# 1005088h/3d_object_detection

Hardware: AMD Instinct MI355X
Metric: point-cloud frames/sec end-to-end (voxelise→NMS), eight_20cm, 1x MI355X (higher is better)
Workload: dtype f32; 1 GPU; configs/eight_20cm.json, synthetic KITTI-shape 64-beam 20k-point clouds (mean 20000 points, one distinct cloud per frame of a step), independent frames (batch=1 semantics), random-init weights (InstanceNorm backbone), AABB NMS; `value`: clouds resident in HBM; frames_per_pass_per_gpu=32, engine_max_batch=32, parallelism=frame-sharded x1

## Files before the change

### 3d_object_detection_amd/csrc/anchor_mask.hip

```cpp
#include "pp_common.h"

namespace {

__device__ __forceinline__ void occ_mark_body(const int32_t* __restrict__ coors, const int32_t* __restrict__ num_pillars,
                                                int gy, int32_t* __restrict__ occ)
{
    int p = blockIdx.x * blockDim.x + threadIdx.x;
    if (p >= *num_pillars) return;
    atomicAdd(&occ[coors[3 * p] * gy + coors[3 * p + 1]], 1);
}

__device__ __forceinline__ void scan_rows_body(int32_t* __restrict__ occ, int gx, int gy)
{
    int row = blockIdx.x * 4 + (threadIdx.x >> 6);
    int lane = threadIdx.x & 63;
    if (row >= gx) return;
    int32_t* r = occ + (size_t)row * gy;
    int carry = 0;
    constexpr int NB = 8;
    for (int yb = 0; yb < gy; yb += 64 * NB) {
        int vv[NB];
#pragma unroll
        for (int b = 0; b < NB; ++b) {
            const int y = yb + b * 64 + lane;
            const int x = r[y < gy ? y : gy - 1];
            vv[b] = y < gy ? x : 0;
        }
#pragma unroll
        for (int b = 0; b < NB; ++b) {
            const int y = yb + b * 64 + lane;
            int v = vv[b];
#pragma unroll
            for (int o = 1; o < 64; o <<= 1) {
                int t = __shfl_up(v, o);
                if (lane >= o) v += t;
            }
            v += carry;
            if (y < gy) r[y] = v;
            carry = __shfl(v, 63);
        }
    }
}

__device__ __forceinline__ void scan_cols_body(int32_t* __restrict__ occ, int gx, int gy)
{
    __shared__ int part[16][64];
    int lane = threadIdx.x & 63, w = threadIdx.x >> 6;
    int col = blockIdx.x * 64 + lane;
    int rows_per = (gx + 15) / 16;
    int x0 = w * rows_per, x1 = min(gx, x0 + rows_per);
    constexpr int CH = 16;
    int s = 0;
    if (col < gy)
        for (int x = x0; x < x1; x += CH) {
            int v[CH];
#pragma unroll
            for (int i = 0; i < CH; ++i) v[i] = occ[(size_t)min(x + i, x1 - 1) * gy + col];
#pragma unroll
            for (int i = 0; i < CH; ++i) s += (x + i < x1) ? v[i] : 0;
        }
    part[w][lane] = s;
    __syncthreads();
    int run = 0;
    for (int k = 0; k < w; ++k) run += part[k][lane];
    if (col < gy)
        for (int x = x0; x < x1; x += CH) {
            int v[CH];
#pragma unroll
            for (int i = 0; i < CH; ++i) v[i] = occ[(size_t)min(x + i, x1 - 1) * gy + col];
#pragma unroll
            for (int i = 0; i < CH; ++i)
                if (x + i < x1) {
                    run += v[i];
                    occ[(size_t)(x + i) * gy + col] = run;
                }
        }
}

__device__ __forceinline__ void mask_lookup_sep_body(const int32_t* __restrict__ sat, int gy, int H, int W, int types,
                                                       const int32_t* __restrict__ rect_x, const int32_t* __restrict__ rect_y,
                                                       uint8_t* __restrict__ mask)
{
    int64_t a = (int64_t)blockIdx.x * blockDim.x + threadIdx.x;
    int64_t total = (int64_t)types * H * W;
    if (a >= total) return;
    int iy = (int)(a % W);
    int64_t q = a / W;
    int ix = (int)(q % H);
    int t = (int)(q / H);
    int minx = rect_x[(t * H + ix) * 2], maxx = rect_x[(t * H + ix) * 2 + 1];
    int miny = rect_y[(t * W + iy) * 2], maxy = rect_y[(t * W + iy) * 2 + 1];
    int area = sat[maxx * gy + maxy] - sat[maxx * gy + miny] - sat[minx * gy + maxy] + sat[minx * gy + miny];
    mask[a] = area > 0;
}

__device__ __forceinline__ void mask_lookup_full_body(const int32_t* __restrict__ sat, int gy, int64_t A,
                                                        const int4* __restrict__ rects, uint8_t* __restrict__ mask)
{
    int64_t a = (int64_t)blockIdx.x * blockDim.x + threadIdx.x;
    if (a >= A) return;
    int4 r = rects[a];
    int area = sat[r.z * gy + r.w] - sat[r.z * gy + r.y] - sat[r.x * gy + r.w] + sat[r.x * gy + r.y];
    mask[a] = area > 0;
}

template <class Src> __global__ void __launch_bounds__(256) occ_mark(Src src, int gy)
{
    const pp_pre_frame F = src.get();
    occ_mark_body(F.coors, F.num, gy, F.occ);
}
template <class Src> __global__ void __launch_bounds__(256) scan_rows(Src src, int gx, int gy) { scan_rows_body(src.get().occ, gx, gy); }
template <class Src> __global__ void __launch_bounds__(1024) scan_cols(Src src, int gx, int gy) { scan_cols_body(src.get().occ, gx, gy); }
template <class Src> __global__ void __launch_bounds__(256) mask_lookup_sep(Src src, int gy, int H, int W, int types, const int32_t* __restrict__ rect_x,
                                                                            const int32_t* __restrict__ rect_y)
{
    const pp_pre_frame F = src.get();
    mask_lookup_sep_body(F.occ, gy, H, W, types, rect_x, rect_y, F.mask);
}
template <class Src> __global__ void __launch_bounds__(256) mask_lookup_full(Src src, int gy, int64_t A, const int4* __restrict__ rects)
{
    const pp_pre_frame F = src.get();
    mask_lookup_full_body(F.occ, gy, A, rects, F.mask);
}

}

template <class Src> static int anchor_mask_stages(pp_ctx* ctx, Src src, int g, hipStream_t stream)
{
    const int gx = ctx->gx, gy = ctx->gy;
    hipLaunchKernelGGL(occ_mark<Src>, dim3(pp_div_up(ctx->cfg.max_voxels, 256), 1, g), dim3(256), 0, stream, src, gy);
    hipLaunchKernelGGL(scan_rows<Src>, dim3(pp_div_up(gx, 4), 1, g), dim3(256), 0, stream, src, gx, gy);
    hipLaunchKernelGGL(scan_cols<Src>, dim3(pp_div_up(gy, 64), 1, g), dim3(1024), 0, stream, src, gx, gy);
    if (ctx->rect_separable) {
        int types = (int)(ctx->A / ((int64_t)ctx->H * ctx->W));
        hipLaunchKernelGGL(mask_lookup_sep<Src>, dim3(pp_div_up(ctx->A, 256), 1, g), dim3(256), 0, stream, src, gy, ctx->H, ctx->W, types,
                           ctx->rect_x, ctx->rect_y);
    } else {
        hipLaunchKernelGGL(mask_lookup_full<Src>, dim3(pp_div_up(ctx->A, 256), 1, g), dim3(256), 0, stream, src, gy, ctx->A, (const int4*)ctx->rects);
    }
    PP_HIP(hipGetLastError());
    return 0;
}

extern "C" int pp_anchor_mask(pp_ctx* ctx, const int32_t* coors, const int32_t* num_pillars, uint8_t* mask, void* stream_)
{
    if (!ctx) return PP_E_ARG;
    if (!coors || !num_pillars || !mask) return pp_fail(ctx, PP_E_ARG, "pp_anchor_mask: null pointer");
    if (ctx->A == 0) return pp_fail(ctx, PP_E_STATE, "pp_anchor_mask: call pp_set_anchors first");
    hipStream_t stream = (hipStream_t)stream_;
    pp_pre_frame f = {};
    PP_SET(f.coors, coors); PP_SET(f.num, num_pillars); PP_SET(f.mask, mask); PP_SET(f.occ, ctx->slot[0].occ);
    PP_HIP(hipMemsetAsync(ctx->slot[0].occ, 0, (size_t)ctx->gx * ctx->gy * sizeof(int32_t), stream));
    return anchor_mask_stages(ctx, pp_frames_one<pp_pre_frame>{f}, 1, stream);
}

int pp_anchor_mask_group(pp_ctx* ctx, int b0, int g, hipStream_t stream)
{
    return anchor_mask_stages(ctx, pp_frames_tab<pp_pre_frame>{ctx->d_pre + b0}, g, stream);
}
```

### 3d_object_detection_amd/csrc/pp_api.hip

```cpp
#include <cmath>
#include <cstdio>
#include <cstdlib>
#include <cstring>
#include "pp_common.h"

static std::string g_create_err;

int pp_fail_hip(pp_ctx* ctx, hipError_t e, const char* what, const char* file, int line)
{
    char buf[512];
    snprintf(buf, sizeof(buf), "%s failed: %s (%s:%d)", what, hipGetErrorString(e), file, line);
    if (ctx) ctx->err = buf; else g_create_err = buf;
    (void)hipGetLastError();
    return -(int)e;
}

int pp_fail(pp_ctx* ctx, int code, const char* msg)
{
    if (ctx) ctx->err = msg; else g_create_err = msg;
    return code;
}

extern "C" const char* pp_last_error(pp_ctx* ctx) { return ctx ? ctx->err.c_str() : g_create_err.c_str(); }
extern "C" int pp_version(void) { return 4; }

int pp_stage_mark(pp_ctx* ctx, hipStream_t stream, int id)
{
    if (!ctx->stage_on) return 0;
    if (ctx->stage_used >= ctx->stage_ev.size()) {
        hipEvent_t e;
        PP_HIP(hipEventCreate(&e));
        ctx->stage_ev.push_back(e);
        ctx->stage_id.push_back(-1);
        ctx->stage_stream.push_back(nullptr);
    }
    const hipError_t er = hipEventRecord(ctx->stage_ev[ctx->stage_used], stream);
    if (er != hipSuccess) { ctx->stage_on = false; ctx->stage_used = 0; return pp_fail_hip(ctx, er, "hipEventRecord(stage mark)", __FILE__, __LINE__); }
    ctx->stage_id[ctx->stage_used] = id;
    ctx->stage_stream[ctx->stage_used] = stream;
    ctx->stage_used++;
    return 0;
}

extern "C" int pp_stage_profile_begin(pp_ctx* ctx)
{
    if (!ctx) return PP_E_ARG;
    ctx->stage_on = true;
    ctx->stage_used = 0;
    return 0;
}

extern "C" int pp_stage_profile_end(pp_ctx* ctx, double* ms_h)
{
    if (!ctx || !ms_h) return PP_E_ARG;
    ctx->stage_on = false;
    const size_t used = ctx->stage_used;
    ctx->stage_used = 0;
    for (int i = 0; i < PP_ST_COUNT; ++i) ms_h[i] = 0.0;
    for (size_t i = 0; i + 1 < used; ++i) {
        const int id = ctx->stage_id[i];
        if (id < 0 || id >= PP_ST_COUNT) continue;
        if (ctx->stage_stream[i] != ctx->stage_stream[i + 1]) continue;
        PP_HIP(hipEventSynchronize(ctx->stage_ev[i]));
        PP_HIP(hipEventSynchronize(ctx->stage_ev[i + 1]));
        float ms = 0.f;
        PP_HIP(hipEventElapsedTime(&ms, ctx->stage_ev[i], ctx->stage_ev[i + 1]));
        ms_h[id] += ms;
    }
    return 0;
}

template <typename T>
static hipError_t dalloc(T** p, size_t count)
{
    return hipMalloc((void**)p, count * sizeof(T) + 256);
}

static int create_impl(pp_ctx* ctx)
{
    const pp_config& c = ctx->cfg;
    PP_HIP(hipSetDevice(ctx->device));
    size_t cells = (size_t)c.grid_size[0] * c.grid_size[1] * c.grid_size[2];
    size_t mp = (size_t)c.max_points;
    ctx->slot.resize(ctx->max_batch);
    for (int b = 0; b < ctx->max_batch; ++b) {
        pp_slot& S = ctx->slot[b];
        const size_t nslots = (size_t)c.max_voxels * c.max_num_points;
        PP_HIP(dalloc(&S.cell_first, cells + nslots + 4));
        S.slots = S.cell_first + cells;
        S.vox_scalars = S.slots + nslots;
        PP_HIP(dalloc(&S.pt_cell, mp));
        PP_HIP(dalloc(&S.pt_rank, mp));
        PP_HIP(dalloc(&S.wave_cnt, mp / 64 + 8));
        PP_HIP(dalloc(&S.occ, (size_t)ctx->gx * ctx->gy));
    }
    PP_HIP(hipMalloc((void**)&ctx->d_pre, sizeof(pp_pre_frame) * ctx->max_batch));
    PP_HIP(hipMalloc((void**)&ctx->d_post, sizeof(pp_post_frame) * ctx->max_batch));
    PP_HIP(dalloc(&ctx->pfn_w, 9 * 64));
    PP_HIP(dalloc(&ctx->pfn_scale, 64));
    PP_HIP(dalloc(&ctx->pfn_shift, 64));
    size_t mv = (size_t)c.max_voxels * ctx->max_batch;
    PP_HIP(dalloc(&ctx->f_voxels, mv * c.max_num_points * c.num_point_features));
    PP_HIP(dalloc(&ctx->f_coors, mv * 3));
    PP_HIP(dalloc(&ctx->f_npts, mv));
    PP_HIP(dalloc(&ctx->f_num, 4 * (size_t)ctx->max_batch));
    PP_HIP(dalloc(&ctx->f_feat, mv * 64));
    PP_HIP(dalloc(&ctx->f_canvas, (size_t)64 * ctx->gx * ctx->gy));
    PP_HIP(dalloc(&ctx->f_pmap, (size_t)ctx->max_batch * ctx->gx * ctx->gy));
    size_t HW = (size_t)ctx->H * ctx->W;
    size_t Amax = HW * c.num_anchor_per_loc * ctx->max_batch;
    PP_HIP(dalloc(&ctx->f_mask, Amax));
    PP_HIP(dalloc(&ctx->f_cls, Amax));
    PP_HIP(dalloc(&ctx->f_box, Amax * 7));
    PP_HIP(dalloc(&ctx->f_dir, Amax * 2));
    int rc = pp_net_create(ctx);
    if (rc) return rc;
    rc = pp_sc1_create(ctx);
    if (rc) return rc;
    rc = pp_ts_create(ctx);
    if (rc) return rc;
    rc = pp_post_create(ctx);
    return rc;
}

extern "C" pp_ctx* pp_create(int device, const pp_config* cfg)
{
    if (!cfg) { pp_fail(nullptr, PP_E_ARG, "pp_create: null config"); return nullptr; }
    if (cfg->grid_size[2] != 1 || cfg->grid_size[0] < 2 || cfg->grid_size[1] < 2 || (cfg->grid_size[0] & 1) ||
        (cfg->grid_size[1] & 1)) {
        pp_fail(nullptr, PP_E_ARG, "pp_create: grid must be [gx,gy,1] with even gx,gy (multiples of 8 for the backbone)");
        return nullptr;
    }
    if (cfg->max_voxels <= 0 || cfg->max_num_points <= 0 || cfg->max_points <= 0 || cfg->num_classes <= 0 ||
        cfg->num_classes > PP_MAX_CLASSES || cfg->max_batch < 0 || cfg->max_batch > 64) {
        pp_fail(nullptr, PP_E_ARG, "pp_create: size out of range");
        return nullptr;
    }
    if (cfg->nms_pre_max <= 0 || cfg->nms_pre_max > 4096) {
        pp_fail(nullptr, PP_E_ARG, "pp_create: nms_pre_max must be in [1, 4096]");
        return nullptr;
    }
    if (cfg->nms_post_max <= 0 || cfg->nms_post_max > 1024) {
        pp_fail(nullptr, PP_E_ARG, "pp_create: nms_post_max must be in [1, 1024]");
        return nullptr;
    }
    if (cfg->nms_post_max > cfg->nms_pre_max) {
        pp_fail(nullptr, PP_E_ARG, "pp_create: nms_post_max must not exceed nms_pre_max");
        return nullptr;
    }
    if (!(cfg->score_threshold > 0.f && cfg->score_threshold < 1.f)) {
        pp_fail(nullptr, PP_E_ARG, "pp_create: score_threshold must be in (0,1)");
        return nullptr;
    }
    pp_ctx* ctx = new pp_ctx();
    ctx->cfg = *cfg;
    ctx->max_batch = cfg->max_batch > 0 ? cfg->max_batch : 1;
    ctx->cfg.max_batch = ctx->max_batch;
    ctx->device = device;
    ctx->gx = cfg->grid_size[0];
    ctx->gy = cfg->grid_size[1];
    ctx->H = ctx->gx / 2;
    ctx->W = ctx->gy / 2;
    if (const char* e = getenv("PP_HEAD_DEFER")) ctx->head_defer_env_off = e[0] == '0';
    ctx->head_defer = !ctx->head_defer_env_off;
    if (const char* e = getenv("PP_SPARSE_CONV1")) ctx->sparse_conv1_env_off = e[0] == '0';
    ctx->sparse_conv1 = !ctx->sparse_conv1_env_off;
    if (const char* e = getenv("PP_TILE_SKIP")) ctx->tile_skip_env_off = e[0] == '0';
    ctx->tile_skip = !ctx->tile_skip_env_off;
    int rc = create_impl(ctx);
    if (rc) {
        g_create_err = ctx->err;
        pp_destroy(ctx);
        return nullptr;
    }
    return ctx;
}

int pp_build_tables(pp_ctx* ctx)
{
    if (ctx->tab_A == ctx->A) return 0;
    const pp_config& c = ctx->cfg;
    const size_t mv = (size_t)c.max_voxels;
    const size_t vs = mv * c.max_num_points * c.num_point_features;
    const size_t cells = (size_t)ctx->gx * ctx->gy;
    const size_t A = (size_t)ctx->A;
    std::vector<pp_pre_frame> pre(ctx->max_batch);
    std::vector<pp_post_frame> post(ctx->max_batch);
    for (int b = 0; b < ctx->max_batch; ++b) {
        const pp_slot& S = ctx->slot[b];
        pp_pre_frame& f = pre[b];
        PP_SET(f.pt_cell, S.pt_cell); PP_SET(f.cell_first, S.cell_first); PP_SET(f.wave_cnt, S.wave_cnt); PP_SET(f.pt_rank, S.pt_rank);
        PP_SET(f.slots, S.slots); PP_SET(f.scalars, S.vox_scalars); PP_SET(f.occ, S.occ);
        PP_SET(f.voxels, ctx->f_voxels + b * vs);
        PP_SET(f.coors, ctx->f_coors + b * mv * 3);
        PP_SET(f.npts, ctx->f_npts + b * mv);
        PP_SET(f.num, ctx->f_num + b * 4);
        PP_SET(f.mask, ctx->f_mask + b * A);
        PP_SET(f.feat, ctx->f_feat + b * mv * 64);
        PP_SET(f.pmap, ctx->f_pmap + b * cells);
        pp_post_frame& q = post[b];
        PP_SET(q.cls, ctx->f_cls + b * A); PP_SET(q.box, ctx->f_box + b * A * 7); PP_SET(q.dir, ctx->f_dir + b * A * 2); PP_SET(q.mask, ctx->f_mask + b * A);
        pp_post_fill_table(ctx, b, &q);
    }
    PP_HIP(hipMemcpy(ctx->d_pre, pre.data(), sizeof(pp_pre_frame) * pre.size(), hipMemcpyHostToDevice));
    PP_HIP(hipMemcpy(ctx->d_post, post.data(), sizeof(pp_post_frame) * post.size(), hipMemcpyHostToDevice));
    ctx->tab_A = ctx->A;
    return 0;
}

extern "C" void pp_destroy(pp_ctx* ctx)
{
    if (!ctx) return;
    (void)hipSetDevice(ctx->device);
    pp_net_destroy(ctx);
    pp_sc1_destroy(ctx);
    pp_ts_destroy(ctx);
    pp_post_destroy(ctx);
    pp_assign_destroy(ctx);
    pp_train_destroy(ctx);
    pp_neck_destroy(ctx);
    pp_block_destroy(ctx);
    pp_down_destroy(ctx);
    pp_pfn_train_destroy(ctx);
    pp_optim_destroy(ctx);
    pp_image16_destroy(ctx);
    for (pp_slot& S : ctx->slot) {
        void* sp[] = {S.cell_first, S.pt_cell, S.pt_rank, S.wave_cnt, S.occ};
        for (void* q : sp)
            if (q) (void)hipFree(q);
    }
    if (ctx->d_pre) (void)hipFree(ctx->d_pre);
    if (ctx->d_post) (void)hipFree(ctx->d_post);
    void* ptrs[] = {ctx->anchors, ctx->rect_x, ctx->rect_y, ctx->rects, ctx->pfn_w, ctx->pfn_scale, ctx->pfn_shift,
                    ctx->f_voxels, ctx->f_coors, ctx->f_npts, ctx->f_num, ctx->f_feat, ctx->f_canvas, ctx->f_mask, ctx->f_pmap,
                    ctx->f_cls, ctx->f_box, ctx->f_dir};
    for (void* p : ptrs)
        if (p) (void)hipFree(p);
    for (hipEvent_t e : ctx->prof_ev) (void)hipEventDestroy(e);
    for (hipEvent_t e : ctx->stage_ev) (void)hipEventDestroy(e);
    delete ctx;
}

extern "C" int pp_set_precision(pp_ctx* ctx, int mode)
{
    if (!ctx || mode < 0 || mode > 4) return pp_fail(ctx, PP_E_ARG, "pp_set_precision: mode must be 0 (fp32), 1 (bf16x3), 2 (bf16), 3 (fp16) or 4 (fp16s)");
    if (ctx->precision != mode) ctx->weights_ready = false;
    ctx->precision = mode;
    return 0;
}

extern "C" int pp_set_train_chunk_frames(pp_ctx* ctx, int k)
{
    if (!ctx) return PP_E_ARG;
    if (k < 0) return pp_fail(ctx, PP_E_ARG, "pp_set_train_chunk_frames: k must be >= 0 (0: the workspace rule alone)");
    ctx->train_chunk_frames = k;
    return 0;
}

extern "C" int pp_load_weights(pp_ctx* ctx, const char* name, const void* host_ptr, const int64_t* shape, int ndim)
{
    if (!ctx || !name || !host_ptr || !shape || ndim < 0 || ndim > 4) return pp_fail(ctx, PP_E_ARG, "pp_load_weights: bad argument");
    pp_tensor_h t;
    int64_t n = 1;
    for (int i = 0; i < ndim; ++i) { t.shape.push_back(shape[i]); n *= shape[i]; }
    if (n <= 0 || n > (1 << 26)) return pp_fail(ctx, PP_E_ARG, "pp_load_weights: bad shape");
    t.data.assign((const float*)host_ptr, (const float*)host_ptr + n);
    ctx->host_w[name] = std::move(t);
    ctx->weights_ready = false;
    return 0;
}

static const pp_tensor_h* find_w(pp_ctx* ctx, const std::string& k, int64_t numel)
{
    auto it = ctx->host_w.find(k);
    if (it == ctx->host_w.end() || (int64_t)it->second.data.size() != numel) return nullptr;
    return &it->second;
}

extern "C" int pp_commit_weights(pp_ctx* ctx)
{
    if (!ctx) return PP_E_ARG;
    PP_HIP(hipSetDevice(ctx->device));
    if (ctx->head_stale && ctx->net) {
        if (int rc0 = pp_head_materialise(ctx, ctx->stale_stream)) return rc0;
        PP_HIP(hipStreamSynchronize(ctx->stale_stream));
    }
    const std::string p = "pillar_point_net.pfn_layers.";
    const pp_tensor_h *w = find_w(ctx, p + "0.weight", 64 * 9), *g = find_w(ctx, p + "1.weight", 64),
                      *b = find_w(ctx, p + "1.bias", 64), *rm = find_w(ctx, p + "1.running_mean", 64),
                      *rv = find_w(ctx, p + "1.running_var", 64);
    if (!w || !g || !b || !rm || !rv) return pp_fail(ctx, PP_E_NAME, "pp_commit_weights: PFN tensors missing or mis-shaped");
    float wT[9 * 64], sc[64], sh[64];
    for (int c = 0; c < 64; ++c) {
        for (int k = 0; k < 9; ++k) wT[k * 64 + c] = w->data[c * 9 + k];
        double s = (double)g->data[c] / std::sqrt((double)rv->data[c] + 1e-5);
        sc[c] = (float)s;
        sh[c] = (float)((double)b->data[c] - (double)rm->data[c] * s);
    }
    PP_HIP(hipMemcpy(ctx->pfn_w, wT, sizeof(wT), hipMemcpyHostToDevice));
    PP_HIP(hipMemcpy(ctx->pfn_scale, sc, sizeof(sc), hipMemcpyHostToDevice));
    PP_HIP(hipMemcpy(ctx->pfn_shift, sh, sizeof(sh), hipMemcpyHostToDevice));
    int rc = pp_net_commit(ctx);
    if (rc) return rc;
    if ((rc = pp_sc1_commit(ctx))) return rc;
    ctx->weights_ready = true;
    ++ctx->commit_gen;
    return 0;
}

extern "C" int pp_set_anchors(pp_ctx* ctx, const float* anchors_h, const int32_t* rects_h, int64_t A)
{
    if (!ctx || !anchors_h || !rects_h || A <= 0) return pp_fail(ctx, PP_E_ARG, "pp_set_anchors: bad argument");
    PP_HIP(hipSetDevice(ctx->device));
    const int H = ctx->H, W = ctx->W;
    const int64_t HW = (int64_t)H * W;
    if (A % HW != 0 || A / HW != ctx->cfg.num_anchor_per_loc)
        return pp_fail(ctx, PP_E_ARG, "pp_set_anchors: A must be num_anchor_per_loc * (gx/2) * (gy/2)");
    for (int i = 0; i < 4 * A; ++i) {
        int lim = (i & 1) ? ctx->gy : ctx->gx;
        if (rects_h[i] < 0 || rects_h[i] >= lim) return pp_fail(ctx, PP_E_ARG, "pp_set_anchors: rectangle outside the grid");
    }
    for (void** q : {(void**)&ctx->anchors, (void**)&ctx->rects, (void**)&ctx->rect_x, (void**)&ctx->rect_y})
        if (*q) { (void)hipFree(*q); *q = nullptr; }
    PP_HIP(dalloc(&ctx->anchors, (size_t)A * 7));
    PP_HIP(hipMemcpy(ctx->anchors, anchors_h, (size_t)A * 7 * sizeof(float), hipMemcpyHostToDevice));
    PP_HIP(dalloc(&ctx->rects, (size_t)A * 4));
    PP_HIP(hipMemcpy(ctx->rects, rects_h, (size_t)A * 4 * sizeof(int32_t), hipMemcpyHostToDevice));
    const int types = (int)(A / HW);
    std::vector<int32_t> rx((size_t)types * H * 2), ry((size_t)types * W * 2);
    bool sep = true;
    for (int t = 0; t < types && sep; ++t)
        for (int ix = 0; ix < H && sep; ++ix)
            for (int iy = 0; iy < W; ++iy) {
                const int32_t* r = rects_h + 4 * (((int64_t)t * H + ix) * W + iy);
                if (iy == 0) { rx[((size_t)t * H + ix) * 2] = r[0]; rx[((size_t)t * H + ix) * 2 + 1] = r[2]; }
                if (ix == 0) { ry[((size_t)t * W + iy) * 2] = r[1]; ry[((size_t)t * W + iy) * 2 + 1] = r[3]; }
                if (r[0] != rx[((size_t)t * H + ix) * 2] || r[2] != rx[((size_t)t * H + ix) * 2 + 1] ||
                    r[1] != ry[((size_t)t * W + iy) * 2] || r[3] != ry[((size_t)t * W + iy) * 2 + 1]) { sep = false; break; }
            }
    ctx->rect_separable = sep ? 1 : 0;
    if (sep) {
        PP_HIP(dalloc(&ctx->rect_x, rx.size()));
        PP_HIP(dalloc(&ctx->rect_y, ry.size()));
        PP_HIP(hipMemcpy(ctx->rect_x, rx.data(), rx.size() * sizeof(int32_t), hipMemcpyHostToDevice));
        PP_HIP(hipMemcpy(ctx->rect_y, ry.data(), ry.size() * sizeof(int32_t), hipMemcpyHostToDevice));
    }
    ctx->A = A;
    return 0;
}
```

### 3d_object_detection_amd/csrc/pp_common.h

```cpp
#pragma once
#include <hip/hip_runtime.h>
#include <stdint.h>
#include <map>
#include <string>
#include <vector>
#include "../../include/pp_hip.h"

#define PP_EMPTY 0x7F7F7F7F

#define PP_HIP(call)                                                         \
    do {                                                                     \
        hipError_t e_ = (call);                                              \
        if (e_ != hipSuccess) return pp_fail_hip(ctx, e_, #call, __FILE__, __LINE__); \
    } while (0)

#if defined(__HIP_DEVICE_COMPILE__)
#define PP_GP __attribute__((address_space(1)))
#else
#define PP_GP
#endif
#define PP_SET(dst, src) dst = (decltype(dst))(src)
struct pp_pre_frame {
    int32_t PP_GP *pt_cell, *cell_first, *wave_cnt, *pt_rank, *slots, *scalars, *occ;
    float PP_GP* voxels;
    int32_t PP_GP *coors, *npts, *num;
    uint8_t PP_GP* mask;
    float PP_GP* feat;
    int32_t PP_GP* pmap;
};
struct pp_post_frame {
    const float PP_GP *cls, *box, *dir;
    const uint8_t PP_GP* mask;
    uint64_t PP_GP *cand, *shortl, *sel, *nmask;
    int32_t PP_GP *counters, *hist, *dirl;
    float PP_GP *boxes, *nbox;
};
template <class F> struct pp_frames_tab {
    const F* tab;
    __device__ F at(int fr) const { return tab[fr]; }
    __device__ F get() const { return tab[blockIdx.z]; }
};
template <class F> struct pp_frames_one {
    F f;
    __device__ F at(int) const { return f; }
    __device__ F get() const { return f; }
};
#define PP_GROUP 32
struct pp_in_group {
    const float* pts[PP_GROUP];
    int32_t n[PP_GROUP];
};

struct pp_tensor_h {
    std::vector<int64_t> shape;
    std::vector<float> data;
};

struct pp_layer {
    float* w = nullptr;
    int cin = 0, cout = 0;
    int ks = 1, stride = 1;
    int up = 1;
    float* bn_scale = nullptr;
    float* bn_shift = nullptr;
};

struct pp_slot {
    int32_t* cell_first = nullptr;
    int32_t* pt_cell = nullptr;
    int32_t* pt_rank = nullptr;
    int32_t* wave_cnt = nullptr;
    int32_t* slots = nullptr;
    int32_t* vox_scalars = nullptr;
    int32_t* occ = nullptr;
    void* post = nullptr;
};

struct pp_ctx {
    pp_config cfg;
    int device = 0;
    std::string err;
    int gx = 0, gy = 0, H = 0, W = 0;
    int max_batch = 1;
    int64_t A = 0;
    std::vector<pp_slot> slot;
    pp_pre_frame* d_pre = nullptr;
    pp_post_frame* d_post = nullptr;
    int64_t tab_A = -1;
    float* anchors = nullptr;
    int32_t* rect_x = nullptr;
    int32_t* rect_y = nullptr;
    int32_t* rects = nullptr;
    int rect_separable = 0;
    float* f_voxels = nullptr; int32_t* f_coors = nullptr; int32_t* f_npts = nullptr; int32_t* f_num = nullptr;
    float* f_feat = nullptr; float* f_canvas = nullptr; uint8_t* f_mask = nullptr; int32_t* f_pmap = nullptr;
    float* f_cls = nullptr; float* f_box = nullptr; float* f_dir = nullptr;
    std::map<std::string, pp_tensor_h> host_w;
    bool weights_ready = false;
    float* pfn_w = nullptr;
    float* pfn_scale = nullptr;
    float* pfn_shift = nullptr;
    void* net = nullptr;
    int precision = 0;
    bool prof_on = false;
    std::vector<hipEvent_t> prof_ev;
    size_t prof_used = 0;
    double prof_flops = 0.0;
    bool stage_on = false;
    std::vector<hipEvent_t> stage_ev;
    std::vector<int> stage_id;
    std::vector<hipStream_t> stage_stream;
    size_t stage_used = 0;
    int last_nb = 0;
    bool asg_thr_set = false;
    float asg_thr_m[PP_MAX_CLASSES] = {}, asg_thr_u[PP_MAX_CLASSES] = {};
    void* asg = nullptr;
    uint64_t commit_gen = 0;
    void* trn = nullptr;
    void* neck = nullptr;
    void* blk = nullptr;
    void* down = nullptr;
    void* pfnt = nullptr;
    void* img16 = nullptr;
    void* optim = nullptr;
    int train_chunk_frames = 0;
    bool head_defer = true;
    bool head_defer_env_off = false;
    bool head_stale = false;
    int stale_nb = 0;
    hipStream_t stale_stream = nullptr;
    bool sparse_conv1 = true;
    bool sparse_conv1_env_off = false;
    void* sc1 = nullptr;
    int sc1_kc = 4;
    int sc1_last_nb = 0;
    bool tile_skip = true;
    bool tile_skip_env_off = false;
    void* ts = nullptr;
    std::vector<int> prof_ts_layer;
    double prof_items = 0.0, prof_items_dense = 0.0;
};
enum { PP_ST_VOXELIZE = 0, PP_ST_MASK = 1, PP_ST_PFN = 2, PP_ST_CONV = 3, PP_ST_NORM = 4, PP_ST_HEAD = 5, PP_ST_POST = 6 ,
       PP_ST_POST_TOPK = 7 , PP_ST_POST_NMS = 8 , PP_ST_COUNT = 12 };
int pp_stage_mark(pp_ctx* ctx, hipStream_t stream, int id);

int pp_fail_hip(pp_ctx* ctx, hipError_t e, const char* what, const char* file, int line);
int pp_fail(pp_ctx* ctx, int code, const char* msg);

int pp_net_create(pp_ctx* ctx);
void pp_net_destroy(pp_ctx* ctx);
int pp_net_commit(pp_ctx* ctx);
int pp_post_create(pp_ctx* ctx);
int pp_run_backbone(pp_ctx* ctx, const float* canvas, int nb, hipStream_t stream, const int32_t* pmap, const float* feat);
int pp_pillar_map(pp_ctx* ctx, const int32_t* coors, const int32_t* num_pillars, int32_t* pmap, hipStream_t stream);
int pp_build_tables(pp_ctx* ctx);
void pp_post_fill_table(pp_ctx* ctx, int slot, pp_post_frame* f);
int pp_voxelize_group(pp_ctx* ctx, int b0, int g, const pp_in_group& in, hipStream_t stream);
int pp_anchor_mask_group(pp_ctx* ctx, int b0, int g, hipStream_t stream);
int pp_pfn_pmap_group(pp_ctx* ctx, int b0, int g, hipStream_t stream);
int pp_postprocess_group(pp_ctx* ctx, int b0, int g, float* det, int32_t* det_count, int nms_mode, hipStream_t stream,
                         int defer_nb = 0);
int pp_run_head_fused(pp_ctx* ctx, float* cls, float* box, float* dir, int nb, hipStream_t stream);
bool pp_head_defer_on(pp_ctx* ctx);
int pp_run_head_cls(pp_ctx* ctx, float* cls, int nb, hipStream_t stream);
int pp_head_materialise(pp_ctx* ctx, hipStream_t stream);
struct pp_head_gather {
    const float* w; int bm, bmp, K;
    const float* bias_perm;
    const float* in; size_t in_fs; int HW;
    int pre; const double* pre_acc; size_t pre_fs; double pre_inv_n; const float *pre_scale, *pre_shift; size_t aff_fs; float eps;
};
int pp_net_head_gather(pp_ctx* ctx, int nb, pp_head_gather* g);
int pp_sc1_create(pp_ctx* ctx);
void pp_sc1_destroy(pp_ctx* ctx);
int pp_sc1_commit(pp_ctx* ctx);
int pp_sc1_update(pp_ctx* ctx, const float* w, hipStream_t stream);
const float* pp_first_conv_image(pp_ctx* ctx, size_t* bytes);
bool pp_sc1_usable(pp_ctx* ctx);
int pp_sc1_run(pp_ctx* ctx, const int32_t* pmap, const float* feat, float* out, double* stat, size_t stat_fs, int nb, hipStream_t stream);
int pp_sc1_fetch_list(pp_ctx* ctx, int frame, void* dst, hipStream_t stream);
const uint64_t* pp_sc1_words(pp_ctx* ctx, int* nblk);
int pp_ts_create(pp_ctx* ctx);
void pp_ts_destroy(pp_ctx* ctx);
bool pp_ts_usable(pp_ctx* ctx, int level0_layers);
void pp_ts_begin_pass(pp_ctx* ctx);
int pp_ts_build(pp_ctx* ctx, int nb, const uint64_t* words, hipStream_t stream);
int pp_ts_build_from_bitmap(pp_ctx* ctx, int nb, const uint8_t* bitmap, hipStream_t stream);
void pp_ts_mark_pass(pp_ctx* ctx, int nb);
void pp_ts_begin_hook(pp_ctx* ctx, bool builds);
void pp_ts_end_hook(pp_ctx* ctx);
bool pp_ts_list(pp_ctx* ctx, int k, int nb, const int2** items, const int32_t** count);
int pp_ts_fill(pp_ctx* ctx, int k, int nb, float* out, size_t out_fs, int C, hipStream_t stream);
int pp_ts_dense_items(pp_ctx* ctx, int nb);
int pp_ts_read_count(pp_ctx* ctx, int k, int32_t* n);
int pp_ts_fetch_flags(pp_ctx* ctx, int frame, void* dst, hipStream_t stream);
void pp_post_destroy(pp_ctx* ctx);
void pp_assign_destroy(pp_ctx* ctx);
void pp_train_destroy(pp_ctx* ctx);
struct pp_head_image {
    float *w = nullptr, *bias = nullptr, *bias_perm = nullptr;
    std::vector<int32_t> wmap, bmap, bpmap;
};
int pp_net_head_image(pp_ctx* ctx, pp_head_image* img, bool any_plan = false);
int pp_net_head_bias(pp_ctx* ctx, pp_head_image* img);
struct pp_layer_image {
    float* w = nullptr;
    size_t elems = 0;
    std::vector<int32_t> wmap;
};
int pp_net_deconv_image(pp_ctx* ctx, int branch, pp_layer_image* img, bool any_plan = false);
void pp_neck_destroy(pp_ctx* ctx);
struct pp_block_image {
    float* w = nullptr;
    int C = 0, T = 0;
    int rows = 0;
    std::vector<int32_t> pmap;
};
int pp_net_conv_image(pp_ctx* ctx, int k, pp_block_image* img, bool any_plan = false);
void pp_block_destroy(pp_ctx* ctx);
void pp_down_destroy(pp_ctx* ctx);
void pp_pfn_train_destroy(pp_ctx* ctx);
void pp_optim_destroy(pp_ctx* ctx);
int pp_update_conv_image(pp_ctx* ctx, int k, const float* w, hipStream_t stream, bool any_plan = false);

struct pp_image16 {
    void* w = nullptr;
    size_t bytes = 0;
    bool is16 = false, fp16 = false;
    std::vector<int32_t> map;
};
int pp_net_layer_index(pp_ctx* ctx, int kind, int ordinal);
int pp_net_image16(pp_ctx* ctx, int layer, pp_image16* img);
int pp_update_image16(pp_ctx* ctx, int layer, const float* s0, const float* s1, const float* s2, int n0, int n1, int n2, hipStream_t stream,
                      bool* is16);
void pp_image16_destroy(pp_ctx* ctx);
int pp_mp_mode_check(pp_ctx* ctx, const char* who, int mode);

static inline int pp_chunk_frames(const pp_ctx* ctx, size_t budget, size_t frame_bytes, int nb, int chunk_frames)
{
    int fc = (int)(budget / frame_bytes);
    fc = fc < 1 ? 1 : fc > nb ? nb : fc;
    if (chunk_frames > 0 && chunk_frames < fc) fc = chunk_frames;
    if (ctx->train_chunk_frames > 0 && ctx->train_chunk_frames < fc) fc = ctx->train_chunk_frames;
    return fc;
}

static inline int pp_div_up(int64_t a, int64_t b) { return (int)((a + b - 1) / b); }
```

### 3d_object_detection_amd/csrc/voxelize.hip

```cpp
#include "pp_common.h"

namespace {

__device__ __forceinline__ int cell_of(const float* __restrict__ p, float ox, float oy, float oz, float vx,
                                       float vy, float vz, int gx, int gy, int gz, int& cx, int& cy, int& cz)
{
    float fx = floorf(__fdiv_rn(__fsub_rn(p[0], ox), vx));
    float fy = floorf(__fdiv_rn(__fsub_rn(p[1], oy), vy));
    float fz = floorf(__fdiv_rn(__fsub_rn(p[2], oz), vz));
    bool in = (fx >= 0.f) & (fx < (float)gx) & (fy >= 0.f) & (fy < (float)gy) & (fz >= 0.f) & (fz < (float)gz);
    if (!in) return -1;
    cx = (int)fx; cy = (int)fy; cz = (int)fz;
    return (cx * gy + cy) * gz + cz;
}

__device__ __forceinline__ void vox_cell_first_body(const float* __restrict__ pts, int n, int nfeat, pp_config cfg,
                                                      int32_t* __restrict__ pt_cell, int32_t* __restrict__ cell_first)
{
    int i = blockIdx.x * blockDim.x + threadIdx.x;
    if (i >= n) return;
    int cx, cy, cz;
    int c = cell_of(pts + (size_t)i * nfeat, cfg.offset[0], cfg.offset[1], cfg.offset[2], cfg.voxel_size[0],
                    cfg.voxel_size[1], cfg.voxel_size[2], cfg.grid_size[0], cfg.grid_size[1], cfg.grid_size[2], cx, cy, cz);
    pt_cell[i] = c;
    if (c >= 0) atomicMin(&cell_first[c], i);
}

__device__ __forceinline__ void vox_flag_count_body(const int32_t* __restrict__ pt_cell,
                                                      const int32_t* __restrict__ cell_first, int n,
                                                      int32_t* __restrict__ wave_cnt)
{
    int i = blockIdx.x * blockDim.x + threadIdx.x;
    bool flag = false;
    if (i < n) {
        int c = pt_cell[i];
        flag = (c >= 0) && (cell_first[c] == i);
    }
    unsigned long long b = __ballot(flag);
    if ((threadIdx.x & 63) == 0) wave_cnt[i >> 6] = __popcll(b);
}

__device__ __forceinline__ void vox_rank_body(const float* __restrict__ pts, int n, int nfeat, pp_config cfg,
                                                const int32_t* __restrict__ pt_cell,
                                                const int32_t* __restrict__ cell_first,
                                                const int32_t* __restrict__ wave_cnt, int32_t* __restrict__ pt_rank,
                                                int32_t* __restrict__ coors, int32_t* __restrict__ scalars,
                                                int32_t* __restrict__ num_pillars)
{
    int i = blockIdx.x * blockDim.x + threadIdx.x;
    int lane = threadIdx.x & 63;
    int w = i >> 6;
    int nw = (n + 63) >> 6;
    int part = 0, tot = 0;
    for (int k = lane; k < nw; k += 64) {
        int v = wave_cnt[k];
        tot += v;
        if (k < w) part += v;
    }
#pragma unroll
    for (int o = 32; o > 0; o >>= 1) {
        part += __shfl_xor(part, o);
        tot += __shfl_xor(tot, o);
    }
    bool flag = false;
    int c = -1;
    if (i < n) {
        c = pt_cell[i];
        flag = (c >= 0) && (cell_first[c] == i);
    }
    unsigned long long b = __ballot(flag);
    int rank = part + __popcll(b & ((1ull << lane) - 1ull));
    if (flag) {
        pt_rank[i] = rank;
        if (rank < cfg.max_voxels) {
            int gy = cfg.grid_size[1], gz = cfg.grid_size[2];
            int cz = c % gz, cy = (c / gz) % gy, cx = c / (gz * gy);
            coors[3 * rank + 0] = cx;
            coors[3 * rank + 1] = cy;
            coors[3 * rank + 2] = cz;
        } else if (rank == cfg.max_voxels) {
            scalars[0] = i;
        }
    }
    if (i == 0) {
        scalars[1] = tot;
        *num_pillars = tot < cfg.max_voxels ? tot : cfg.max_voxels;
    }
}

__device__ __forceinline__ void vox_insert_body(int n, pp_config cfg, const int32_t* __restrict__ pt_cell,
                                                  const int32_t* __restrict__ cell_first,
                                                  const int32_t* __restrict__ pt_rank,
                                                  const int32_t* __restrict__ scalars, int32_t* __restrict__ slots)
{
    int i = blockIdx.x * blockDim.x + threadIdx.x;
    if (i >= n || i >= scalars[0]) return;
    int c = pt_cell[i];
    if (c < 0) return;
    int r = pt_rank[cell_first[c]];
    if (r >= cfg.max_voxels) return;
    int32_t* s = slots + (size_t)r * cfg.max_num_points;
    int x = i;
    for (int k = 0; k < cfg.max_num_points; ++k) {
        int old = atomicMin(&s[k], x);
        x = old > x ? old : x;
        if (x >= PP_EMPTY) break;
    }
}

__device__ __forceinline__ void vox_gather_body(const float* __restrict__ pts, int nfeat, pp_config cfg,
                                                  const int32_t* __restrict__ slots,
                                                  const int32_t* __restrict__ num_pillars, float* __restrict__ voxels,
                                                  int32_t* __restrict__ npts)
{
    int t = blockIdx.x * blockDim.x + threadIdx.x;
    int T = cfg.max_num_points;
    int p = t / T, k = t - p * T;
    if (p >= *num_pillars) return;
    int idx = slots[t];
    bool have = idx < PP_EMPTY;
    float* dst = voxels + (size_t)t * nfeat;
    if (nfeat == 4) {
        float4 v = have ? *reinterpret_cast<const float4*>(pts + (size_t)idx * 4) : make_float4(0.f, 0.f, 0.f, 0.f);
        *reinterpret_cast<float4*>(dst) = v;
    } else {
        for (int f = 0; f < nfeat; ++f) dst[f] = have ? pts[(size_t)idx * nfeat + f] : 0.f;
    }
    if (k == 0) {
        int cnt = 0;
        for (int q = 0; q < T; ++q) cnt += slots[(size_t)p * T + q] < PP_EMPTY;
        npts[p] = cnt;
    }
}

template <class Src> __global__ void __launch_bounds__(256) vox_cell_first(pp_in_group in, Src src, int nfeat, pp_config cfg)
{
    const pp_pre_frame F = src.get();
    vox_cell_first_body(in.pts[blockIdx.z], in.n[blockIdx.z], nfeat, cfg, F.pt_cell, F.cell_first);
}
template <class Src> __global__ void __launch_bounds__(256) vox_flag_count(pp_in_group in, Src src)
{
    const pp_pre_frame F = src.get();
    vox_flag_count_body(F.pt_cell, F.cell_first, in.n[blockIdx.z], F.wave_cnt);
}
template <class Src> __global__ void __launch_bounds__(256) vox_rank(pp_in_group in, Src src, int nfeat, pp_config cfg)
{
    const pp_pre_frame F = src.get();
    vox_rank_body(in.pts[blockIdx.z], in.n[blockIdx.z], nfeat, cfg, F.pt_cell, F.cell_first, F.wave_cnt, F.pt_rank, F.coors, F.scalars, F.num);
}
template <class Src> __global__ void __launch_bounds__(256) vox_insert(pp_in_group in, Src src, pp_config cfg)
{
    const pp_pre_frame F = src.get();
    vox_insert_body(in.n[blockIdx.z], cfg, F.pt_cell, F.cell_first, F.pt_rank, F.scalars, F.slots);
}
template <class Src> __global__ void __launch_bounds__(256) vox_gather(pp_in_group in, Src src, int nfeat, pp_config cfg)
{
    const pp_pre_frame F = src.get();
    vox_gather_body(in.pts[blockIdx.z], nfeat, cfg, F.slots, F.num, F.voxels, F.npts);
}

__global__ void __launch_bounds__(256) pre_init_b(const pp_pre_frame* __restrict__ tab, int n7f, int nocc, int npmap)
{
    const pp_pre_frame F = tab[blockIdx.z];
    const int stride = gridDim.x * blockDim.x;
    for (int i = blockIdx.x * blockDim.x + threadIdx.x; i < n7f; i += stride) F.cell_first[i] = PP_EMPTY;
    for (int i = blockIdx.x * blockDim.x + threadIdx.x; i < nocc; i += stride) F.occ[i] = 0;
    for (int i = blockIdx.x * blockDim.x + threadIdx.x; i < npmap; i += stride) F.pmap[i] = -1;
}

}

template <class Src> static int voxelize_stages(pp_ctx* ctx, Src src, int g, const pp_in_group& in, int nmax, hipStream_t stream)
{
    const pp_config& cfg = ctx->cfg;
    const int nfeat = cfg.num_point_features;
    const int nb = pp_div_up(nmax > 0 ? nmax : 1, 256);
    hipLaunchKernelGGL(vox_cell_first<Src>, dim3(nb, 1, g), dim3(256), 0, stream, in, src, nfeat, cfg);
    hipLaunchKernelGGL(vox_flag_count<Src>, dim3(nb, 1, g), dim3(256), 0, stream, in, src);
    hipLaunchKernelGGL(vox_rank<Src>, dim3(nb, 1, g), dim3(256), 0, stream, in, src, nfeat, cfg);
    hipLaunchKernelGGL(vox_insert<Src>, dim3(nb, 1, g), dim3(256), 0, stream, in, src, cfg);
    const int nt = cfg.max_voxels * cfg.max_num_points;
    hipLaunchKernelGGL(vox_gather<Src>, dim3(pp_div_up(nt, 256), 1, g), dim3(256), 0, stream, in, src, nfeat, cfg);
    PP_HIP(hipGetLastError());
    return 0;
}

static size_t vox_fill_words(const pp_config& cfg)
{
    return (size_t)cfg.grid_size[0] * cfg.grid_size[1] * cfg.grid_size[2] + (size_t)cfg.max_voxels * cfg.max_num_points + 4;
}

extern "C" int pp_voxelize(pp_ctx* ctx, const float* pts, int n, int nfeat, float* voxels, int32_t* coors,
                           int32_t* npts, int32_t* num_pillars, void* stream_)
{
    if (!ctx) return PP_E_ARG;
    hipStream_t stream = (hipStream_t)stream_;
    const pp_slot& S = ctx->slot[0];
    const pp_config& cfg = ctx->cfg;
    if (n < 0 || n > cfg.max_points) return pp_fail(ctx, PP_E_ARG, "pp_voxelize: n exceeds cfg.max_points");
    if (nfeat != cfg.num_point_features || nfeat < 3) return pp_fail(ctx, PP_E_ARG, "pp_voxelize: nfeat mismatch");
    if (!voxels || !coors || !npts || !num_pillars || (n > 0 && !pts)) return pp_fail(ctx, PP_E_ARG, "pp_voxelize: null pointer");
    if (n == 0) {
        PP_HIP(hipMemsetAsync(num_pillars, 0, sizeof(int32_t), stream));
        return 0;
    }
    pp_pre_frame f = {};
    PP_SET(f.pt_cell, S.pt_cell); PP_SET(f.cell_first, S.cell_first); PP_SET(f.wave_cnt, S.wave_cnt); PP_SET(f.pt_rank, S.pt_rank);
    PP_SET(f.slots, S.slots); PP_SET(f.scalars, S.vox_scalars);
    PP_SET(f.voxels, voxels); PP_SET(f.coors, coors); PP_SET(f.npts, npts); PP_SET(f.num, num_pillars);
    pp_in_group in = {};
    in.pts[0] = pts;
    in.n[0] = n;
    PP_HIP(hipMemsetAsync(S.cell_first, 0x7F, vox_fill_words(cfg) * sizeof(int32_t), stream));
    return voxelize_stages(ctx, pp_frames_one<pp_pre_frame>{f}, 1, in, n, stream);
}

int pp_voxelize_group(pp_ctx* ctx, int b0, int g, const pp_in_group& in, hipStream_t stream)
{
    const pp_config& cfg = ctx->cfg;
    int nmax = 0;
    for (int i = 0; i < g; ++i) {
        if (in.n[i] < 0 || in.n[i] > cfg.max_points) return pp_fail(ctx, PP_E_ARG, "pp_infer_batch: n exceeds cfg.max_points");
        if (in.n[i] > 0 && !in.pts[i]) return pp_fail(ctx, PP_E_ARG, "pp_infer_batch: null point cloud");
        nmax = in.n[i] > nmax ? in.n[i] : nmax;
    }
    const pp_pre_frame* tab = ctx->d_pre + b0;
    const int nbev = ctx->gx * ctx->gy;
    hipLaunchKernelGGL(pre_init_b, dim3(256, 1, g), dim3(256), 0, stream, tab, (int)vox_fill_words(cfg), nbev, nbev);
    return voxelize_stages(ctx, pp_frames_tab<pp_pre_frame>{tab}, g, in, nmax, stream);
}

namespace {
struct pp_pc2_fields { int32_t off[4]; int32_t dt[4]; };

__global__ void __launch_bounds__(256) pc2_unpack(const uint8_t* __restrict__ data, int64_t n, int64_t width, int64_t row_step, int point_step,
                                                  pp_pc2_fields f, int big_endian, float* __restrict__ out)
{
    const int64_t t = (int64_t)blockIdx.x * blockDim.x + threadIdx.x;
    if (t >= n * 4) return;
    const int64_t i = t >> 2;
    const int k = (int)(t & 3);
    const uint8_t* src = data + (i / width) * row_step + (i % width) * point_step + f.off[k];
    const int dt = f.dt[k];
    const int nbytes = (dt == 1 || dt == 2) ? 1 : (dt == 3 || dt == 4) ? 2 : (dt == 8) ? 8 : 4;
    uint64_t bits = 0;
    for (int b = 0; b < nbytes; ++b) {
        const uint64_t byte = src[b];
        bits |= byte << (8 * (big_endian ? (nbytes - 1 - b) : b));
    }
    float val;
    switch (dt) {
    case 1: val = (float)(int8_t)bits; break;
    case 2: val = (float)(uint8_t)bits; break;
    case 3: val = (float)(int16_t)bits; break;
    case 4: val = (float)(uint16_t)bits; break;
    case 5: val = (float)(int32_t)bits; break;
    case 6: val = (float)(uint32_t)bits; break;
    case 8: val = (float)__longlong_as_double((long long)bits); break;
    default: val = __uint_as_float((uint32_t)bits); break;
    }
    out[t] = val;
}
}

extern "C" int pp_unpack_points(const void* data, int64_t n, int64_t width, int64_t row_step, int point_step, const int32_t* offs,
                                const int32_t* dtypes, int big_endian, float* out, void* stream)
{
    if (n < 0 || width <= 0 || point_step <= 0 || row_step < 0 || !offs || !dtypes) return PP_E_ARG;
    if (n == 0) return 0;
    if (!data || !out) return PP_E_ARG;
    pp_pc2_fields f;
    for (int k = 0; k < 4; ++k) {
        if (dtypes[k] < 1 || dtypes[k] > 8 || offs[k] < 0) return PP_E_ARG;
        const int nb = (dtypes[k] <= 2) ? 1 : (dtypes[k] <= 4) ? 2 : (dtypes[k] == 8) ? 8 : 4;
        if (offs[k] + nb > point_step) return PP_E_ARG;
        f.off[k] = offs[k];
        f.dt[k] = dtypes[k];
    }
    hipLaunchKernelGGL(pc2_unpack, dim3(pp_div_up(n * 4, 256)), dim3(256), 0, (hipStream_t)stream, (const uint8_t*)data, n, width, row_step,
                       point_step, f, big_endian, out);
    hipError_t e = hipGetLastError();
    return e == hipSuccess ? 0 : -(int)e;
}
```

Measured before the change: 1093 frames/s.

## Compute anchor mask from occupancy bitmaps instead of summed-area table

Replaces the int32 occupancy grid, its row and column prefix scans, and the per-anchor SAT lookup with a 64-bit occupancy bitmap. A per-distinct-y-rectangle pass ORs bit ranges into y-bitmasks, and an expand pass ORs those over each x range and writes 16 mask bytes per thread. This removes two full-grid scan kernels and cuts zero-init traffic from 4 bytes to 1 bit per cell. In exchange it adds a dedup step over y-rectangle classes on the host, and it only applies when the rectangles are separable and ordered with at most 32 types.

Measured after the change: 1094 frames/s (median of 4 runs). Within noise of the previous version (+0.1%).

```diff
diff --git a/3d_object_detection_amd/csrc/anchor_mask.hip b/3d_object_detection_amd/csrc/anchor_mask.hip
--- a/3d_object_detection_amd/csrc/anchor_mask.hip
+++ b/3d_object_detection_amd/csrc/anchor_mask.hip
@@ -104,6 +104,76 @@
     mask[a] = area > 0;
 }
 
+constexpr int YROWS = 16;
+
+__device__ __forceinline__ void occ_mark_bits_body(const int32_t* __restrict__ coors, const int32_t* __restrict__ num_pillars, int gx, int gy,
+                                                     uint64_t* __restrict__ bits)
+{
+    int p = blockIdx.x * blockDim.x + threadIdx.x;
+    if (p >= *num_pillars) return;
+    const int x = coors[3 * p], y = coors[3 * p + 1];
+    if ((unsigned)x < (unsigned)gx && (unsigned)y < (unsigned)gy)
+        atomicOr((unsigned long long*)&bits[(size_t)x * ((gy + 63) >> 6) + (y >> 6)], 1ull << (y & 63));
+}
+
+__device__ __forceinline__ void mask_ybits_body(const uint64_t* __restrict__ bits, int gx, int wpr, int W, int nwy, int d, int wy,
+                                                  const int32_t* __restrict__ ry , uint64_t* __restrict__ ybits)
+{
+    const int lane = threadIdx.x & 63, wave = threadIdx.x >> 6;
+    const int iy = wy * 64 + lane;
+    int lo = 1, hi = 0;
+    if (iy < W) { lo = ry[iy * 2] + 1; hi = ry[iy * 2 + 1]; }
+    const int wlo = lo >> 6, whi = hi >> 6;
+    const uint64_t mlo = ~0ull << (lo & 63), mhi = ~0ull >> (63 - (hi & 63));
+    const int x0 = (blockIdx.x * 4 + wave) * YROWS;
+    if (x0 >= gx) return;
+    uint32_t any = 0;
+    for (int w = wlo; w <= whi; ++w) {
+        const uint64_t m = (w == wlo ? mlo : ~0ull) & (w == whi ? mhi : ~0ull);
+        uint64_t v[YROWS];
+#pragma unroll
+        for (int r = 0; r < YROWS; ++r) v[r] = bits[(size_t)min(x0 + r, gx - 1) * wpr + w];
+#pragma unroll
+        for (int r = 0; r < YROWS; ++r) any |= (uint32_t)((v[r] & m) != 0) << r;
+    }
+#pragma unroll
+    for (int r = 0; r < YROWS; ++r) {
+        const uint64_t word = __ballot((any >> r) & 1);
+        if (lane == 0 && x0 + r < gx) ybits[((size_t)d * gx + x0 + r) * nwy + wy] = word;
+    }
+}
+
+__device__ __forceinline__ void mask_expand_body(const uint64_t* __restrict__ yb , int nwy, int H, int W, int t,
+                                                   const int32_t* __restrict__ rect_x, uint8_t PP_GP* mask)
+{
+    const int nseg = (W + 15) >> 4;
+    const int i = blockIdx.x * blockDim.x + threadIdx.x;
+    if (i >= H * nseg) return;
+    const int seg = i % nseg, ix = i / nseg;
+    const int minx = rect_x[(t * H + ix) * 2], maxx = rect_x[(t * H + ix) * 2 + 1];
+    const uint64_t* y = yb + (seg >> 2);
+    uint64_t acc = 0;
+    constexpr int CH = 8;
+    for (int x = minx + 1; x <= maxx; x += CH) {
+        uint64_t v[CH];
+#pragma unroll
+        for (int k = 0; k < CH; ++k) v[k] = y[(size_t)min(x + k, maxx) * nwy];
+#pragma unroll
+        for (int k = 0; k < CH; ++k) acc |= v[k];
+    }
+    const uint32_t b16 = (uint32_t)(acc >> ((seg & 3) * 16)) & 0xFFFFu;
+    uint32_t o[4];
+#pragma unroll
+    for (int j = 0; j < 4; ++j) o[j] = (((b16 >> (4 * j)) & 0xFu) * 0x00204081u) & 0x01010101u;
+    const int iy0 = seg * 16;
+    uint8_t PP_GP* dst = mask + ((int64_t)t * H + ix) * W + iy0;
+    if (iy0 + 16 <= W && ((uintptr_t)dst & 15) == 0) {
+        *(uint4 PP_GP*)dst = make_uint4(o[0], o[1], o[2], o[3]);
+    } else {
+        for (int k = 0; k < 16 && iy0 + k < W; ++k) dst[k] = (uint8_t)((b16 >> k) & 1u);
+    }
+}
+
 template <class Src> __global__ void __launch_bounds__(256) occ_mark(Src src, int gy)
 {
     const pp_pre_frame F = src.get();
@@ -122,7 +192,37 @@
     const pp_pre_frame F = src.get();
     mask_lookup_full_body(F.occ, gy, A, rects, F.mask);
 }
-
+template <class Src> __global__ void __launch_bounds__(256) occ_mark_bits(Src src, int gx, int gy)
+{
+    const pp_pre_frame F = src.get();
+    occ_mark_bits_body(F.coors, F.num, gx, gy, F.occ_bits);
+}
+template <class Src> __global__ void __launch_bounds__(256) mask_ybits(Src src, int gx, int wpr, int W, int nwy, pp_ycls yc, const int32_t* __restrict__ rect_y)
+{
+    const pp_pre_frame F = src.get();
+    const int d = blockIdx.y / nwy, wy = blockIdx.y % nwy;
+    mask_ybits_body(F.occ_bits, gx, wpr, W, nwy, d, wy, rect_y + (size_t)yc.rep[d] * W * 2, F.ybits);
+}
+template <class Src> __global__ void __launch_bounds__(256) mask_expand(Src src, int gx, int nwy, int H, int W, pp_ycls yc, const int32_t* __restrict__ rect_x)
+{
+    const pp_pre_frame F = src.get();
+    const int t = blockIdx.y;
+    mask_expand_body(F.ybits + (size_t)yc.of[t] * gx * nwy, nwy, H, W, t, rect_x, F.mask);
+}
+
+}
+
+template <class Src> static int anchor_mask_bit_stages(pp_ctx* ctx, Src src, int g, hipStream_t stream)
+{
+    const int gx = ctx->gx, gy = ctx->gy, H = ctx->H, W = ctx->W;
+    const int wpr = pp_div_up(gy, 64), nwy = pp_div_up(W, 64), types = (int)(ctx->A / ((int64_t)H * W));
+    hipLaunchKernelGGL(occ_mark_bits<Src>, dim3(pp_div_up(ctx->cfg.max_voxels, 256), 1, g), dim3(256), 0, stream, src, gx, gy);
+    hipLaunchKernelGGL(mask_ybits<Src>, dim3(pp_div_up(gx, 4 * YROWS), ctx->ycls.D * nwy, g), dim3(256), 0, stream, src, gx, wpr, W, nwy, ctx->ycls,
+                       ctx->rect_y);
+    hipLaunchKernelGGL(mask_expand<Src>, dim3(pp_div_up((int64_t)H * pp_div_up(W, 16), 256), types, g), dim3(256), 0, stream, src, gx, nwy, H, W,
+                       ctx->ycls, ctx->rect_x);
+    PP_HIP(hipGetLastError());
+    return 0;
 }
 
 template <class Src> static int anchor_mask_stages(pp_ctx* ctx, Src src, int g, hipStream_t stream)
@@ -156,5 +256,6 @@
 
 int pp_anchor_mask_group(pp_ctx* ctx, int b0, int g, hipStream_t stream)
 {
+    if (pp_mask_from_bits(ctx)) return anchor_mask_bit_stages(ctx, pp_frames_tab<pp_pre_frame>{ctx->d_pre + b0}, g, stream);
     return anchor_mask_stages(ctx, pp_frames_tab<pp_pre_frame>{ctx->d_pre + b0}, g, stream);
 }
diff --git a/3d_object_detection_amd/csrc/pp_api.hip b/3d_object_detection_amd/csrc/pp_api.hip
--- a/3d_object_detection_amd/csrc/pp_api.hip
+++ b/3d_object_detection_amd/csrc/pp_api.hip
@@ -93,6 +93,9 @@
         PP_HIP(dalloc(&S.pt_rank, mp));
         PP_HIP(dalloc(&S.wave_cnt, mp / 64 + 8));
         PP_HIP(dalloc(&S.occ, (size_t)ctx->gx * ctx->gy));
+        const size_t nbits = (size_t)ctx->gx * pp_div_up(ctx->gy, 64);
+        PP_HIP(dalloc(&S.occ_bits, nbits + (size_t)c.num_anchor_per_loc * ctx->gx * pp_div_up(ctx->W, 64)));
+        S.ybits = S.occ_bits + nbits;
     }
     PP_HIP(hipMalloc((void**)&ctx->d_pre, sizeof(pp_pre_frame) * ctx->max_batch));
     PP_HIP(hipMalloc((void**)&ctx->d_post, sizeof(pp_post_frame) * ctx->max_batch));
@@ -191,6 +194,7 @@
         pp_pre_frame& f = pre[b];
         PP_SET(f.pt_cell, S.pt_cell); PP_SET(f.cell_first, S.cell_first); PP_SET(f.wave_cnt, S.wave_cnt); PP_SET(f.pt_rank, S.pt_rank);
         PP_SET(f.slots, S.slots); PP_SET(f.scalars, S.vox_scalars); PP_SET(f.occ, S.occ);
+        PP_SET(f.occ_bits, S.occ_bits); PP_SET(f.ybits, S.ybits);
         PP_SET(f.voxels, ctx->f_voxels + b * vs);
         PP_SET(f.coors, ctx->f_coors + b * mv * 3);
         PP_SET(f.npts, ctx->f_npts + b * mv);
@@ -225,7 +229,7 @@
     pp_optim_destroy(ctx);
     pp_image16_destroy(ctx);
     for (pp_slot& S : ctx->slot) {
-        void* sp[] = {S.cell_first, S.pt_cell, S.pt_rank, S.wave_cnt, S.occ};
+        void* sp[] = {S.cell_first, S.pt_cell, S.pt_rank, S.wave_cnt, S.occ, S.occ_bits};
         for (void* q : sp)
             if (q) (void)hipFree(q);
     }
@@ -339,6 +343,17 @@
                     r[1] != ry[((size_t)t * W + iy) * 2] || r[3] != ry[((size_t)t * W + iy) * 2 + 1]) { sep = false; break; }
             }
     ctx->rect_separable = sep ? 1 : 0;
+    ctx->ycls = {};
+    bool ordered = true;
+    for (size_t i = 0; i < rx.size(); i += 2) ordered = ordered && rx[i] <= rx[i + 1];
+    for (size_t i = 0; i < ry.size(); i += 2) ordered = ordered && ry[i] <= ry[i + 1];
+    if (sep && ordered && types <= PP_MAX_TYPES)
+        for (int t = 0; t < types; ++t) {
+            int d = 0;
+            while (d < ctx->ycls.D && memcmp(&ry[(size_t)ctx->ycls.rep[d] * W * 2], &ry[(size_t)t * W * 2], (size_t)W * 2 * sizeof(int32_t))) ++d;
+            if (d == ctx->ycls.D) ctx->ycls.rep[ctx->ycls.D++] = t;
+            ctx->ycls.of[t] = d;
+        }
     if (sep) {
         PP_HIP(dalloc(&ctx->rect_x, rx.size()));
         PP_HIP(dalloc(&ctx->rect_y, ry.size()));
diff --git a/3d_object_detection_amd/csrc/pp_common.h b/3d_object_detection_amd/csrc/pp_common.h
--- a/3d_object_detection_amd/csrc/pp_common.h
+++ b/3d_object_detection_amd/csrc/pp_common.h
@@ -22,6 +22,7 @@
 #define PP_SET(dst, src) dst = (decltype(dst))(src)
 struct pp_pre_frame {
     int32_t PP_GP *pt_cell, *cell_first, *wave_cnt, *pt_rank, *slots, *scalars, *occ;
+    uint64_t PP_GP *occ_bits, *ybits;
     float PP_GP* voxels;
     int32_t PP_GP *coors, *npts, *num;
     uint8_t PP_GP* mask;
@@ -49,6 +50,13 @@
 struct pp_in_group {
     const float* pts[PP_GROUP];
     int32_t n[PP_GROUP];
+};
+
+#define PP_MAX_TYPES 32
+struct pp_ycls {
+    int32_t D;
+    int32_t rep[PP_MAX_TYPES];
+    int32_t of[PP_MAX_TYPES];
 };
 
 struct pp_tensor_h {
@@ -73,6 +81,8 @@
     int32_t* slots = nullptr;
     int32_t* vox_scalars = nullptr;
     int32_t* occ = nullptr;
+    uint64_t* occ_bits = nullptr;
+    uint64_t* ybits = nullptr;
     void* post = nullptr;
 };
 
@@ -92,6 +102,7 @@
     int32_t* rect_y = nullptr;
     int32_t* rects = nullptr;
     int rect_separable = 0;
+    pp_ycls ycls = {};
     float* f_voxels = nullptr; int32_t* f_coors = nullptr; int32_t* f_npts = nullptr; int32_t* f_num = nullptr;
     float* f_feat = nullptr; float* f_canvas = nullptr; uint8_t* f_mask = nullptr; int32_t* f_pmap = nullptr;
     float* f_cls = nullptr; float* f_box = nullptr; float* f_dir = nullptr;
@@ -246,3 +257,4 @@
 }
 
 static inline int pp_div_up(int64_t a, int64_t b) { return (int)((a + b - 1) / b); }
+static inline bool pp_mask_from_bits(const pp_ctx* ctx) { return ctx->rect_separable && ctx->ycls.D > 0; }
diff --git a/3d_object_detection_amd/csrc/voxelize.hip b/3d_object_detection_amd/csrc/voxelize.hip
--- a/3d_object_detection_amd/csrc/voxelize.hip
+++ b/3d_object_detection_amd/csrc/voxelize.hip
@@ -159,12 +159,13 @@
     vox_gather_body(in.pts[blockIdx.z], nfeat, cfg, F.slots, F.num, F.voxels, F.npts);
 }
 
-__global__ void __launch_bounds__(256) pre_init_b(const pp_pre_frame* __restrict__ tab, int n7f, int nocc, int npmap)
+__global__ void __launch_bounds__(256) pre_init_b(const pp_pre_frame* __restrict__ tab, int n7f, int nocc, int nbits, int npmap)
 {
     const pp_pre_frame F = tab[blockIdx.z];
     const int stride = gridDim.x * blockDim.x;
     for (int i = blockIdx.x * blockDim.x + threadIdx.x; i < n7f; i += stride) F.cell_first[i] = PP_EMPTY;
     for (int i = blockIdx.x * blockDim.x + threadIdx.x; i < nocc; i += stride) F.occ[i] = 0;
+    for (int i = blockIdx.x * blockDim.x + threadIdx.x; i < nbits; i += stride) F.occ_bits[i] = 0;
     for (int i = blockIdx.x * blockDim.x + threadIdx.x; i < npmap; i += stride) F.pmap[i] = -1;
 }
 
@@ -226,7 +227,9 @@
     }
     const pp_pre_frame* tab = ctx->d_pre + b0;
     const int nbev = ctx->gx * ctx->gy;
-    hipLaunchKernelGGL(pre_init_b, dim3(256, 1, g), dim3(256), 0, stream, tab, (int)vox_fill_words(cfg), nbev, nbev);
+    const bool bits = pp_mask_from_bits(ctx);
+    hipLaunchKernelGGL(pre_init_b, dim3(256, 1, g), dim3(256), 0, stream, tab, (int)vox_fill_words(cfg), bits ? 0 : nbev,
+                       bits ? ctx->gx * pp_div_up(ctx->gy, 64) : 0, nbev);
     return voxelize_stages(ctx, pp_frames_tab<pp_pre_frame>{tab}, g, in, nmax, stream);
 }
 
```
